# dbandstra/zang

Hardware: AMD Instinct MI355X
Metric: voice-samples/sec (higher is better)
Workload: dtype f32

## Files before the change

### zang_amd/csrc/common.hip.h

```cpp
#pragma once
#if defined(__HIPCC_RTC__)
#define ZH_DEVICE_ONLY 1
#endif
#include <hip/hip_runtime.h>
#if !defined(ZH_DEVICE_ONLY)
#include <stdint.h>
#include <stddef.h>
#include <new>
#endif
#include "rtc_types.hip.h"
#include "../../include/zang_hip.h"

#if !defined(ZH_DEVICE_ONLY)
#include <utility>
#include <vector>
#include <functional>
#include <memory>
#include <string>
struct zh_flipper {
    uint64_t id;
    zh_ctx *ctx;
    uint32_t n;
    uint32_t *cnt[2];
    int cur;
// ... 17 lines not shown
    std::function<void(hipStream_t, float *const *, uint32_t)> launch;
    const char *kernel = nullptr;
};
struct zh_direct_item {
    std::function<void(hipStream_t, float *const *, uint32_t)> launch;
    std::vector<float *> imgs;
    const char *kernel;
};

struct zh_ctx {
    int device;
    hipStream_t stream;
    bool own_stream;
    uint32_t capture_flags;
    bool epoch_open;
    zh_co_batch co;
    uint32_t co_paints, co_launches;
    std::string last_form;
    bool form_fresh;
    float *mix_partials;
    size_t mix_partials_floats;
    std::vector<float *> mix_retired;
    uint32_t graphs_live;
    std::vector<struct zh_graph *> graphs;
    bool capturing;
    uint32_t capture_serial;
    std::vector<zh_flip_use> capture_log;
    std::vector<std::pair<std::string, uint32_t>> capture_kernels;
    int deferred_error = 0;
    std::vector<zh_direct_item> co_plan;
    bool co_plan_ok = true;
    uint32_t capture_launches = 0, co_plan_launches = 0;
    void *noise_jump;
};

struct zh_graph {
    zh_ctx *ctx;
    hipGraph_t graph;
    hipGraphExec_t exec;
    std::vector<zh_flip_use> flips;
    uint32_t nodes = 0;
    uint32_t co_paints = 0, co_launches = 0;
    std::vector<std::pair<std::string, uint32_t>> kernels;
    std::vector<zh_direct_item> plan;
    std::vector<std::pair<std::string, uint32_t>> plan_kernels;
};

struct ZhDeviceGuard {
    int prev, want;
    explicit ZhDeviceGuard(int device) : prev(-1), want(device) {
        if (want < 0) return;
        if (hipGetDevice(&prev) != hipSuccess) { prev = -1; return; }
        if (prev != want) (void)hipSetDevice(want);
    }
    ~ZhDeviceGuard() { if (want >= 0 && prev >= 0 && prev != want) (void)hipSetDevice(prev); }
    ZhDeviceGuard(const ZhDeviceGuard &) = delete;
    ZhDeviceGuard &operator=(const ZhDeviceGuard &) = delete;
};
void zh_epoch_barrier(zh_ctx *ctx);
extern thread_local zh_ctx *zh_tls_ctx;
struct ZhFormScope {
    zh_ctx *prev;
    explicit ZhFormScope(const zh_ctx *c) : prev(zh_tls_ctx) {
        if (!prev) { zh_tls_ctx = const_cast<zh_ctx *>(c); if (zh_tls_ctx) zh_tls_ctx->form_fresh = true; }
    }
    ~ZhFormScope() { zh_tls_ctx = prev; }
};
#define ZH_GUARD_EPOCH(ctxptr) const zh_ctx *_zh_gctx = (ctxptr); ZhDeviceGuard _zh_guard(_zh_gctx ? _zh_gctx->device : -1); ZhFormScope _zh_fscope(_zh_gctx)
#define ZH_LAUNCH(kernel, ...) do { zh_note_launch(zh_tls_ctx, #kernel); hipLaunchKernelGGL(kernel, __VA_ARGS__); } while (0)
#define ZH_GUARD(ctxptr) ZH_GUARD_EPOCH(ctxptr); do { if (_zh_gctx && _zh_gctx->epoch_open) zh_epoch_barrier(const_cast<zh_ctx *>(_zh_gctx)); } while (0)
void zh_epoch_flush_batch(zh_ctx *ctx, bool last);

void zh_flipper_register(zh_flipper *f);
void zh_flipper_unregister(zh_flipper *f);
void zh_flipper_used(zh_flipper *f);
void zh_flipper_painted(zh_flipper *f);

enum { ZF_SINE_RANGES, ZF_NOISE_RANGES, ZF_ENVELOPE_RANGES, ZF_SAMPLER_RANGES, ZF_DECIMATOR_RANGES, ZF_CURVE_RANGES, ZF_CYCLE_RANGES,
       ZF_PORTAMENTO_RANGES, ZF_PULSE_CTRL_RANGES, ZF_PULSE_CTRL_SUMS, ZF_TRISAW_CTRL_RANGES, ZF_TRISAW_CTRL_QUOT, ZF_PMOSC_RANGES,
       ZF_SCRIPT_RANGES, ZF_SCRIPT_RANGES_MAXV, ZF_OSC_FC, ZF_NICE_PC_MAX, ZF_NICE_PC4_MAX, ZF_NICE_WAVE_MAX, ZF_PMOSC_WAVE_MAX,
       ZF_NICE_MIX_ROLL, ZF_NICE_MIX_WG_MIN, ZF_NF_PC_MAX, ZF_NF_RING_MAX, ZF_FILTER_PC_MAX, ZF_FILTER_PC16_MAX, ZF_FILTER_PC_CTL_MAX,
       ZF_PINK_PIPE_MAX, ZF_PINK_TAPS, ZF_ECHOES_PC_MAX, ZF_DELAY_FRAMES_MAX, ZF_FILTER_TP_MAX, ZF_NF_TP_MAX, ZF_NICE_TP_MAX,
       ZF_PINK_TP_MAX, ZF_ECHOES_TP_MAX, ZF_NICE_MIX_FMA, ZF_BASICS_ROWS_MIN, ZF_SCRIPT_PC, ZF_SCRIPT_PC_MAXV, ZF_NF_TP_PIPE_FRAMES, ZF_DISTORTION_ROWS_MIN, ZF_DISTORTION_RC, ZF_GRAPH_DIRECT,
       ZF_STEREO_ECHOES_PC_MAX, ZF_COUNT };
long zh_form(int id);
bool zh_form_is_set(int id);
uint32_t zh_range_frames(uint32_t V, uint32_t n, int form, uint32_t target_waves, uint32_t max_voices);
void zh_note_launch(zh_ctx *ctx, const char *kernel);
extern thread_local const char *zh_tls_launch_detail;

constexpr int kMixGroupFrames = 8;

struct zh_event {
    hipEvent_t ev;
};
#endif

#define ZH_INLINE_LAMBDA __attribute__((always_inline))

#if !defined(ZH_DEVICE_ONLY)
#define ZH_TRY(expr)                                   \
    do {                                               \
        hipError_t _e = (expr);                        \
        if (_e != hipSuccess) return (int)_e;          \
    } while (0)

static inline int zh_launch_status() {
    hipError_t e = hipGetLastError();
    return e == hipSuccess ? ZH_OK : (int)e;
}
#endif

struct Img {
    float *p;
    uint32_t stride;
    __device__ __forceinline__ float *at(uint32_t f, uint32_t v) const { return p + (size_t)f * stride + v; }
};
struct CImg {
    const float *p;
    uint32_t stride;
    __device__ __forceinline__ const float *at(uint32_t f, uint32_t v) const { return p + (size_t)f * stride + v; }
};
struct F32P {
    float value;
    const float *pv;
    __device__ __forceinline__ float get(uint32_t v) const { return pv ? pv[v] : value; }
};
struct BoolP {
    uint32_t value;
    const uint8_t *pv;
    __device__ __forceinline__ bool get(uint32_t v) const { return pv ? pv[v] != 0 : value != 0; }
};
struct CobP {
    uint32_t is_buffer;
    F32P c;
    CImg b;
};

#if !defined(ZH_DEVICE_ONLY)
static inline Img mk_img(const zh_buf &b) { return Img{b.ptr, b.stride}; }
static inline CImg mk_cimg(const zh_buf &b) { return CImg{b.ptr, b.stride}; }
static inline F32P mk_f32(const zh_f32 &f) { return F32P{f.value, f.per_voice}; }
static inline BoolP mk_bool(const zh_bool &b) { return BoolP{b.value, b.per_voice}; }
static inline CobP mk_cob(const zh_cob &c) {
    return CobP{c.tag == ZH_COB_BUFFER ? 1u : 0u, mk_f32(c.constant), mk_cimg(c.buffer)};
}

constexpr uint32_t kMaxRowStride = 1u << 26;
static inline bool buf_covers(const zh_buf &b, uint32_t n_voices, uint32_t span_end) {
    return b.ptr != nullptr && b.voices >= n_voices && b.frames >= span_end && b.stride >= n_voices && b.stride <= kMaxRowStride;
}
static inline bool bufs_alias(const zh_buf &a, const zh_buf &b) {
    if (!a.ptr || !b.ptr) return false;
    const float *ae = a.ptr + (size_t)a.frames * a.stride, *be = b.ptr + (size_t)b.frames * b.stride;
    return a.ptr < be && b.ptr < ae;
}
static inline bool cob_aliases(const zh_cob &c, const zh_buf &b) { return c.tag == ZH_COB_BUFFER && bufs_alias(c.buffer, b); }
static inline int zh_zero_first_aliased(zh_ctx *ctx, uint32_t start, uint32_t end, const zh_buf &out, uint32_t n_voices, bool aliased, uint32_t &flags) {
    if (!aliased || !(flags & ZH_PAINT_ZERO_FIRST)) return ZH_OK;
    flags &= ~(uint32_t)ZH_PAINT_ZERO_FIRST;
    zh_buf o = out;
    o.voices = n_voices;
    return end > start ? zh_zero(ctx, start, end, o) : ZH_OK;
}
static inline bool cob_ok(const zh_cob &c, uint32_t n_voices, uint32_t span_end) {
    if (c.tag == ZH_COB_CONSTANT) return true;
    if (c.tag == ZH_COB_BUFFER) return buf_covers(c.buffer, n_voices, span_end);
// ... 59 lines not shown
```

### zang_amd/csrc/composite.hip

```cpp
#include "common.hip.h"
#include <memory>
#include "ring.hip.h"
#include "zmath.hip.h"
#include "dsp.hip.h"
#include "seq.hip.h"
#include "envelope.hip.h"
#include "voices.hip.h"
#include "span_walk.hip.h"
#include "noise_jump.hip.h"
#define ZH_FILTER_TP_NOISE 1
#include "filter_tp.hip.h"
#include <vector>
#include <string.h>
#include <stdlib.h>

int zh_mix_reserve(zh_ctx *ctx, size_t floats);
void zh_mix_pass2_launch(zh_ctx *ctx, uint32_t tiles, uint32_t nframes, float *dst, int zero_first);
void zh_mix_pass2_launch_at(zh_ctx *ctx, const float *partials, uint32_t tiles, uint32_t nframes, float *dst, int zero_first);
void zh_mix_pass2_wide_launch(zh_ctx *ctx, const float *partials, size_t channel_stride, uint32_t rows, uint32_t nframes, float *dst0,
                              float *dst1, int channels, int zero_first);
void zh_mix_pass2_wide_batch_launch(zh_ctx *ctx, const float *partials, size_t channel_stride, uint32_t rows, uint32_t nframes,
                                    float *const *dst0, float *const *dst1, uint32_t n_buffers, int channels, int zero_first);

struct zh_nice {
// ... 1218 lines not shown
    if (!m || !outputs || !p || end < start || !buf_covers(outputs[0], m->n, end)) return ZH_ERR_INVALID;
    if (m->n == 0) return ZH_OK;
    hipStream_t st = m->ctx->stream;
    NiceArgs a = nice_args(m, p, note_id_changed);
    const Img out = mk_img(outputs[0]);
    const bool zf = (flags & ZH_PAINT_ZERO_FIRST) != 0;
    if ((flags & ZH_PAINT_TOLERANT) && end - start >= 128 && end - start <= kNiceTpMaxChunks * 128u) {
        const uint32_t C = zh_tp_chunks(m->n, ZF_NICE_TP_MAX, end - start);
        if (C >= 2 && !m->tp && !m->ctx->capturing && dev_alloc(&m->tp, (size_t)kNiceTpWords * m->n) != ZH_OK) { m->tp = nullptr; (void)hipGetLastError(); }
        if (C >= 2 && m->tp) {
            NiceTpArgs t;
            t.a = a; t.tp = m->tp; t.start = start; t.end = end; t.L = ((end - start + C - 1) / C + 7) / 8 * 8; t.out = out;
            const dim3 grid((m->n + 255) / 256, (end - start + t.L - 1) / t.L);
            ZH_LAUNCH(k_nice_tp_a, grid, dim3(256), 0, st, t);
            if (zf) ZH_LAUNCH(k_nice_tp_b<true>, grid, dim3(256), 0, st, t);
            else ZH_LAUNCH(k_nice_tp_b<false>, grid, dim3(256), 0, st, t);
            return zh_launch_status();
        }
    }
    if (m->n <= nice_pc_max() && end > start && outputs[0].stride <= (1u << 24)) {
        const long pc4_max = zh_form(ZF_NICE_PC4_MAX);
        if ((long)m->n <= pc4_max) {
            if (zf) ZH_LAUNCH(k_nice_pc4<true>, seq_grid(m->n), dim3(256), 0, st, a, out, start, end);
            else ZH_LAUNCH(k_nice_pc4<false>, seq_grid(m->n), dim3(256), 0, st, a, out, start, end);
        } else {
            if (zf) ZH_LAUNCH(k_nice_pc<true>, seq_grid(m->n), dim3(192), 0, st, a, out, start, end);
            else ZH_LAUNCH(k_nice_pc<false>, seq_grid(m->n), dim3(192), 0, st, a, out, start, end);
        }
    } else {
        if (zf) ZH_LAUNCH((k_nice<true, 1>), seq_grid(m->n), dim3(kSeqBlock), 0, st, a, out, start, end);
        else ZH_LAUNCH((k_nice<false, 1>), seq_grid(m->n), dim3(kSeqBlock), 0, st, a, out, start, end);
    }
    return zh_launch_status();
}
static bool nice_mix_roll() { return zh_form(ZF_NICE_MIX_ROLL) != 0; }
static int nice_mix_wg(uint32_t n_voices) { return (long)n_voices >= zh_form(ZF_NICE_MIX_WG_MIN) ? 4 : 0; }
constexpr uint32_t kNiceCoalesceReserve = 8;
static int nice_paint_mix_n(zh_nice *m, uint32_t start, uint32_t end, float *mix_l, float *mix_r, const zh_f32 *gain_l,
                            const zh_f32 *gain_r, zh_bool note_id_changed, const zh_nice_params *p, uint32_t flags) {
    const bool stereo = mix_r != nullptr;
    if (!m || !mix_l || !p || end < start) return ZH_ERR_INVALID;
    if (m->n == 0) return ZH_OK;
    const uint32_t nframes = end - start;
    const int wg = nice_mix_wg(m->n);
    const uint32_t bs = 256u;
    const uint32_t blocks = (m->n + bs - 1) / bs;
    const uint32_t rows = wg ? blocks : blocks * 4;
    const size_t per_channel = (size_t)rows * kMixGroupFrames * ((nframes + kMixGroupFrames - 1) / kMixGroupFrames ? (nframes + kMixGroupFrames - 1) / kMixGroupFrames : 1);
    int rc = zh_mix_reserve(m->ctx, per_channel * (stereo ? 2 : 1) * (stereo && !m->ctx->capturing ? kNiceCoalesceReserve : 1u));
    if (rc) return rc;
    hipStream_t st = m->ctx->stream;
    NiceArgs a = nice_args(m, p, note_id_changed);
    float *part = m->ctx->mix_partials;
    const int zf = (int)(flags & ZH_PAINT_ZERO_FIRST);
    if ((flags & ZH_PAINT_TOLERANT) && !wg && nframes >= 128 && nframes <= kNiceTpMaxChunks * 128u) {
        const uint32_t Cn = zh_tp_chunks(m->n, ZF_NICE_TP_MAX, nframes);
        if (Cn >= 2 && !m->tp && !m->ctx->capturing && dev_alloc(&m->tp, (size_t)kNiceTpWords * m->n) != ZH_OK) { m->tp = nullptr; (void)hipGetLastError(); }
        if (Cn >= 2 && m->tp) {
            NiceTpArgs t;
            t.a = a; t.tp = m->tp; t.start = start; t.end = end; t.L = ((nframes + Cn - 1) / Cn + MIXF - 1) / MIXF * MIXF; t.out = Img{nullptr, 0};
            const dim3 grid(blocks, (nframes + t.L - 1) / t.L);
            ZH_LAUNCH(k_nice_tp_a, grid, dim3(256), 0, st, t);
            const bool roll = nice_mix_roll();
            if (stereo) {
                const F32P gl = mk_f32(*gain_l), gr = mk_f32(*gain_r);
                if (roll) ZH_LAUNCH((k_nice_mix_tp_b<2, true>), grid, dim3(256), 0, st, t, part, gl, gr);
                else ZH_LAUNCH((k_nice_mix_tp_b<2, false>), grid, dim3(256), 0, st, t, part, gl, gr);
                zh_mix_pass2_wide_launch(m->ctx, part, per_channel, rows, nframes, mix_l + start, mix_r + start, 2, zf);
            } else {
                const F32P none = mk_f32(zh_f32{0.0f, 0, nullptr});
                if (roll) ZH_LAUNCH((k_nice_mix_tp_b<1, true>), grid, dim3(256), 0, st, t, part, none, none);
                else ZH_LAUNCH((k_nice_mix_tp_b<1, false>), grid, dim3(256), 0, st, t, part, none, none);
                zh_mix_pass2_wide_launch(m->ctx, part, per_channel, rows, nframes, mix_l + start, nullptr, 1, zf);
            }
            return zh_launch_status();
        }
    }
    if ((flags & ZH_PAINT_TOLERANT) && zh_form(ZF_NICE_MIX_FMA) != 0) {
        const F32P none = mk_f32(zh_f32{0.0f, 0, nullptr});
        zh_nice_mix_fma_launch(stereo ? 2 : 1, nice_mix_roll(), wg, blocks, st, a, start, end, part, stereo ? mk_f32(*gain_l) : none, stereo ? mk_f32(*gain_r) : none);
        if (nframes) zh_mix_pass2_wide_launch(m->ctx, part, per_channel, rows, nframes, mix_l + start, stereo ? mix_r + start : nullptr, stereo ? 2 : 1, zf);
        return zh_launch_status();
    }
#define ZH_NMIX(C_, ROLL_, NW_, GL_, GR_) ZH_LAUNCH((k_nice_mix<C_, ROLL_, NW_>), dim3(blocks), dim3(bs), 0, st, a, start, end, part, GL_, GR_)
#define ZH_NMIX_W(C_, ROLL_, GL_, GR_) do { if (wg) ZH_NMIX(C_, ROLL_, 4, GL_, GR_); else ZH_NMIX(C_, ROLL_, 0, GL_, GR_); } while (0)
    const bool roll = nice_mix_roll();
    if (stereo) {
        const F32P gl = mk_f32(*gain_l), gr = mk_f32(*gain_r);
        if (roll) ZH_NMIX_W(2, true, gl, gr); else ZH_NMIX_W(2, false, gl, gr);
        if (nframes) zh_mix_pass2_wide_launch(m->ctx, part, per_channel, rows, nframes, mix_l + start, mix_r + start, 2, zf);
    } else {
        const F32P none = mk_f32(zh_f32{0.0f, 0, nullptr});
        if (roll) ZH_NMIX_W(1, true, none, none); else ZH_NMIX_W(1, false, none, none);
        if (nframes) zh_mix_pass2_wide_launch(m->ctx, part, per_channel, rows, nframes, mix_l + start, nullptr, 1, zf);
    }
#undef ZH_NMIX_W
#undef ZH_NMIX
    return zh_launch_status();
}
int zh_nice_paint_mix(zh_nice *m, uint32_t start, uint32_t end, float *mix, zh_bool note_id_changed,
                      const zh_nice_params *p, uint32_t flags) { ZH_GUARD(m ? m->ctx : nullptr);
    return nice_paint_mix_n(m, start, end, mix, nullptr, nullptr, nullptr, note_id_changed, p, flags);
}
constexpr uint32_t kNiceCoalesceMax = 8;
static int nice_paint_mix_batch_impl(zh_nice *m, uint32_t start, uint32_t end, uint32_t n_buffers, float *const *mix_left,
                                     float *const *mix_right, zh_f32 gain_left, zh_f32 gain_right, const zh_bool *note_id_changed,
                                     const zh_nice_params *params, uint32_t flags);
struct NiceHeld { float *l, *r; zh_bool nic; zh_nice_params p; };
struct NiceHeldBatch { std::vector<NiceHeld> v; zh_f32 gl, gr; uint32_t flags, sample_rate_bits; };
static bool same_f32(const zh_f32 &a, const zh_f32 &b) {
    return a.per_voice == b.per_voice && (a.per_voice || __builtin_bit_cast(uint32_t, a.value) == __builtin_bit_cast(uint32_t, b.value));
}
int zh_nice_paint_mix_stereo(zh_nice *m, uint32_t start, uint32_t end, float *mix_left, float *mix_right, zh_f32 gain_left,
                             zh_f32 gain_right, zh_bool note_id_changed, const zh_nice_params *p, uint32_t flags) { ZH_GUARD_EPOCH(m ? m->ctx : nullptr);
    if (!mix_right) return ZH_ERR_INVALID;
    zh_ctx *ctx = m ? m->ctx : nullptr;
    const bool hold = ctx && ctx->capturing && (ctx->capture_flags & ZH_CAPTURE_COALESCE) && mix_left && p && end > start && m->n &&
                      (!(flags & ZH_PAINT_TOLERANT) || nice_mix_wg(m->n));
    bool fits = false;
    if (hold) {
        const uint32_t blocks = (m->n + 255u) / 256u, rows = nice_mix_wg(m->n) ? blocks : blocks * 4;
        const uint32_t groups = (end - start + kMixGroupFrames - 1) / kMixGroupFrames;
        fits = (size_t)rows * kMixGroupFrames * groups * 2 <= ctx->mix_partials_floats;
    }
    if (!hold || !fits) {
        if (ctx && ctx->epoch_open) zh_epoch_barrier(ctx);
        return nice_paint_mix_n(m, start, end, mix_left, mix_right, &gain_left, &gain_right, note_id_changed, p, flags);
    }
    zh_co_batch &cb = ctx->co;
    std::shared_ptr<NiceHeldBatch> held = cb.active && cb.owner == m ? std::static_pointer_cast<NiceHeldBatch>(cb.items) : nullptr;
    const uint32_t sr_bits = __builtin_bit_cast(uint32_t, p->sample_rate);
    bool join = held && cb.start == start && cb.end == end && held->flags == flags && held->sample_rate_bits == sr_bits && held->v.size() < kNiceCoalesceMax &&
                same_f32(held->gl, gain_left) && same_f32(held->gr, gain_right);
    for (size_t q = 0; join && q < held->v.size(); q++) {
        const float *rows[2] = {held->v[q].l, held->v[q].r};
        for (const float *x : rows)
            if ((mix_left < x + end && x < mix_left + end) || (mix_right < x + end && x < mix_right + end)) join = false;
    }
    if (!join) {
        zh_epoch_flush_batch(ctx, false);
        held = std::make_shared<NiceHeldBatch>();
        held->gl = gain_left; held->gr = gain_right; held->flags = flags; held->sample_rate_bits = sr_bits;
        cb.items = held;
        cb.active = true; cb.owner = m; cb.start = start; cb.end = end; cb.stride = 0; cb.key = 0; cb.flips = false;
        ctx->epoch_open = true;
        std::shared_ptr<NiceHeldBatch> items = held;
        cb.launch = [m, start, end, gain_left, gain_right, flags, items](hipStream_t, float *const *, uint32_t cnt) {
            const std::vector<NiceHeld> &v = items->v;
            float *l[kNiceCoalesceMax], *r[kNiceCoalesceMax];
            zh_bool nic[kNiceCoalesceMax];
            zh_nice_params ps[kNiceCoalesceMax];
            for (uint32_t i = 0; i < cnt; i++) { l[i] = v[i].l; r[i] = v[i].r; nic[i] = v[i].nic; ps[i] = v[i].p; }
            int rc = cnt > 1 ? nice_paint_mix_batch_impl(m, start, end, cnt, l, r, gain_left, gain_right, nic, ps, flags) : ZH_ERR_UNSUPPORTED;
            if (rc != ZH_OK) {
                for (uint32_t i = 0; i < cnt; i++) {
                    rc = nice_paint_mix_n(m, start, end, l[i], r[i], &gain_left, &gain_right, nic[i], &ps[i], flags);
                    if (rc != ZH_OK && !m->ctx->deferred_error) m->ctx->deferred_error = rc;
                }
            }
        };
    }
    held->v.push_back(NiceHeld{mix_left, mix_right, note_id_changed, *p});
    cb.imgs.push_back(mix_left);
    ctx->co_paints++;
    return ZH_OK;
}

static int nice_paint_mix_batch_impl(zh_nice *m, uint32_t start, uint32_t end, uint32_t n_buffers, float *const *mix_left,
                                     float *const *mix_right, zh_f32 gain_left, zh_f32 gain_right, const zh_bool *note_id_changed,
                                     const zh_nice_params *params, uint32_t flags) {
    if (!m || !mix_left || !mix_right || !note_id_changed || !params || end < start || n_buffers > (uint32_t)kNiceMixMaxBatch) return ZH_ERR_INVALID;
    for (uint32_t k = 0; k < n_buffers; k++) {
        if (!mix_left[k] || !mix_right[k]) return ZH_ERR_INVALID;
        if (__builtin_bit_cast(uint32_t, params[k].sample_rate) != __builtin_bit_cast(uint32_t, params[0].sample_rate)) return ZH_ERR_UNSUPPORTED;
    }
    if (m->n == 0 || n_buffers == 0) return ZH_OK;
    const uint32_t nframes = end - start;
    const int wg = nice_mix_wg(m->n);
    const uint32_t bs = 256u;
    const uint32_t blocks = (m->n + bs - 1) / bs, rows = wg ? blocks : blocks * 4;
    const size_t per_channel = (size_t)rows * kMixGroupFrames * ((nframes + kMixGroupFrames - 1) / kMixGroupFrames ? (nframes + kMixGroupFrames - 1) / kMixGroupFrames : 1);
    int rc = zh_mix_reserve(m->ctx, per_channel * 2 * n_buffers);
    if (rc) return rc;
    NiceBatchArgs b;
    b.a = nice_args(m, &params[0], note_id_changed[0]);
    b.nb = n_buffers;
    for (int k = 0; k < kNiceMixMaxBatch; k++) {
        const uint32_t j = (uint32_t)k < n_buffers ? (uint32_t)k : 0u;
        b.freq[k] = mk_f32(params[j].freq); b.note_on[k] = mk_bool(params[j].note_on); b.nic[k] = mk_bool(note_id_changed[j]);
    }
    float *part = m->ctx->mix_partials;
    hipStream_t st = m->ctx->stream;
#define ZH_NMIXB(ROLL_, NW_) ZH_LAUNCH((k_nice_mix_batch<2, ROLL_, NW_>), dim3(blocks), dim3(bs), 0, st, b, start, end, part, mk_f32(gain_left), mk_f32(gain_right))
    if ((flags & ZH_PAINT_TOLERANT) && zh_form(ZF_NICE_MIX_FMA) != 0)
        zh_nice_mix_batch_fma_launch(nice_mix_roll(), wg, blocks, st, b, start, end, part, mk_f32(gain_left), mk_f32(gain_right));
    else if (wg) { if (nice_mix_roll()) ZH_NMIXB(true, 4); else ZH_NMIXB(false, 4); }
    else { if (nice_mix_roll()) ZH_NMIXB(true, 0); else ZH_NMIXB(false, 0); }
#undef ZH_NMIXB
    if (nframes) {
        float *l[kNiceMixMaxBatch], *r[kNiceMixMaxBatch];
        for (uint32_t k = 0; k < n_buffers; k++) { l[k] = mix_left[k] + start; r[k] = mix_right[k] + start; }
        zh_mix_pass2_wide_batch_launch(m->ctx, part, per_channel, rows, nframes, l, r, n_buffers, 2, (int)(flags & ZH_PAINT_ZERO_FIRST));
    }
    return zh_launch_status();
}

int zh_nice_paint_mix_stereo_batch(zh_nice *m, uint32_t start, uint32_t end, uint32_t n_buffers, float *const *mix_left,
                                   float *const *mix_right, zh_f32 gain_left, zh_f32 gain_right, const zh_bool *note_id_changed,
                                   const zh_nice_params *params, uint32_t flags) { ZH_GUARD(m ? m->ctx : nullptr);
    return nice_paint_mix_batch_impl(m, start, end, n_buffers, mix_left, mix_right, gain_left, gain_right, note_id_changed, params, flags);
}

static bool span_table_ok(const zh_span_table *t) {
    return t && t->max_spans > 0 && t->count && t->start && t->end && t->freq && t->note_on && t->note_id_changed;
}
static SpanTableP mk_span_table(const zh_span_table *t) {
    return SpanTableP{t->max_spans, t->count, t->start, t->end, t->freq, t->note_on, t->note_id_changed};
}

int zh_nice_paint_spans(zh_nice *m, uint32_t start, uint32_t end, const zh_buf *outputs, const zh_buf *temps,
                        float sample_rate, const zh_span_table *table, uint32_t flags) { ZH_GUARD(m ? m->ctx : nullptr);
    (void)temps;
    if (!m || !outputs || end < start || !buf_covers(outputs[0], m->n, end) || !span_table_ok(table)) return ZH_ERR_INVALID;
    if (m->n == 0) return ZH_OK;
    hipStream_t st = m->ctx->stream;
    zh_nice_params p;
    memset(&p, 0, sizeof p);
    p.sample_rate = sample_rate;
    zh_bool no = {0, 0, nullptr};
    NiceArgs a = nice_args(m, &p, no);
    const bool zf = (flags & ZH_PAINT_ZERO_FIRST) != 0;
    const long wave_max = zh_form(ZF_NICE_WAVE_MAX);
    if ((long)m->n <= wave_max) {
        if (zf) ZH_LAUNCH(k_nice_spans_wave<true>, dim3(m->n), dim3(64), 0, st, a, mk_span_table(table), mk_img(outputs[0]), start, end);
        else ZH_LAUNCH(k_nice_spans_wave<false>, dim3(m->n), dim3(64), 0, st, a, mk_span_table(table), mk_img(outputs[0]), start, end);
    } else if (zf) ZH_LAUNCH(k_nice_spans<true>, seq_grid(m->n), dim3(kSeqBlock), 0, st, a, mk_span_table(table), mk_img(outputs[0]), start, end);
    else ZH_LAUNCH(k_nice_spans<false>, seq_grid(m->n), dim3(kSeqBlock), 0, st, a, mk_span_table(table), mk_img(outputs[0]), start, end);
    return zh_launch_status();
}

int zh_noise_filter_create(zh_ctx *ctx, uint32_t n, uint64_t first_seed, zh_noise_filter **out) { ZH_GUARD(ctx);
    if (!ctx || !out) return ZH_ERR_INVALID;
    zh_noise_filter *m = new (std::nothrow) zh_noise_filter();
    if (!m) return ZH_ERR_INVALID;
    memset(m, 0, sizeof *m);
    m->ctx = ctx; m->n = n;
    int rc = 0;
    for (int i = 0; i < 4 && !rc; i++) rc = dev_alloc(&m->s[i], n);
    if (!rc) rc = dev_alloc(&m->nb, (size_t)7 * n);
    if (!rc) rc = dev_alloc(&m->l, n);
    if (!rc) rc = dev_alloc(&m->b, n);
    if (!rc) rc = dev_alloc(&m->err, 1);
    if (!rc) rc = (int)hipMemsetAsync(m->err, 0, 4, ctx->stream);
    if (!rc && n) {
        rc = (int)hipMemsetAsync(m->nb, 0, (size_t)7 * n * 4, ctx->stream);
        if (!rc) rc = (int)hipMemsetAsync(m->l, 0, (size_t)n * 4, ctx->stream);
        if (!rc) rc = (int)hipMemsetAsync(m->b, 0, (size_t)n * 4, ctx->stream);
    }
    if (rc) { nf_free(m); delete m; return rc; }
    if (n) ZH_LAUNCH(k_nf_seed, dim3((n + 255) / 256), dim3(256), 0, ctx->stream, m->s[0], m->s[1], m->s[2], m->s[3], n, first_seed);
    if (n) (void)zh_noise_jump_tables(ctx);
    *out = m;
    return zh_launch_status();
}
int zh_noise_filter_destroy(zh_noise_filter *m) { ZH_GUARD(m ? m->ctx : nullptr);
    if (!m) return ZH_ERR_INVALID;
    (void)hipStreamSynchronize(m->ctx->stream);
    nf_free(m);
    delete m;
// ... 309 lines not shown
```

### zang_amd/csrc/dispatch.hip

```cpp
#include "common.hip.h"
#include <mutex>
#include <stdlib.h>
#include <string.h>
#include <string>

namespace {
struct FormRow { const char *name; long def; const char *doc; };
const FormRow kForms[ZF_COUNT] = {
     {"sine_ranges", -1, "SineOsc: frame ranges of the span at once, each replaying the phase walk before it (k_sineosc_ranges); auto: ~4,096 waves up to 1 Mi voices, ~2,048 up to 65,536 with a control image"},
     {"noise_ranges", -1, "Noise: frame ranges from jumped generator states (noise_jump.hip); auto: by voice count up to 65,536"},
     {"envelope_ranges", -1, "Envelope: frame ranges, each replaying the clock (k_envelope_ranges); auto: ~2,048 waves up to 40,960 voices"},
     {"sampler_ranges", -1, "Sampler: frame ranges (positions are a product, no replay); auto: ~16,384 waves up to 1 Mi voices"},
     {"decimator_ranges", -1, "Decimator: frame ranges replaying the hold counter; auto: ~1,024-2,048 waves up to 65,536 voices"},
     {"curve_ranges", -1, "Curve: frame ranges; auto: ~2,048 waves up to 40,960 voices"},
     {"cycle_ranges", -1, "Cycle: frame ranges (constant speed); auto: ~1,024 waves up to 16,384 voices"},
     {"portamento_ranges", -1, "Portamento: frame ranges; auto: ~2,048 waves up to 32,768 voices"},
     {"pulse_ctrl_ranges", -1, "PulseOsc with a frequency image: frame ranges over the summed phase advances; auto: ~2,048 waves up to 40,960 voices"},
     {"pulse_ctrl_sums", 1, "... 1: a first kernel sums each range's own advances (k_pulseosc_ctrl_sums), 0: every range replays the frames before it"},
     {"trisaw_ctrl_ranges", -1, "TriSawOsc with a frequency image: frame ranges; auto: ~1,024 waves up to 16,384 voices"},
     {"trisaw_ctrl_quot", 1, "... 1: freq / sample_rate painted once into a module-owned image first (k_div_image), 0: divided in every replay"},
     {"pmosc_ranges", -1, "PMOscInstrument: frame ranges (k_pmosc_ranges); auto: ~2,048-4,096 waves up to 131,072 voices"},
     {"script_ranges", -1, "generated script kernels: frame ranges for modules without a delay ring; auto: by voice count"},
     {"script_ranges_maxv", 131072, "... the largest voice count that takes them"},
     {"osc_fc", 0, "constant-frequency PulseOsc / TriSawOsc: frames per lane of the chunked kernel; 0 = PulseOsc 4, from 16,384 voices 3 with non-temporal stores (profiles/r05/osc_large_voice_counts.txt); TriSawOsc 8-64 by voice count (tools/sweep_osc_fc.sh), PulseOsc's when the paint is a sawtooth for every voice (one color <= 0)"},
     {"nice_pc_max", 65536, "NiceInstrument: up to here the oscillator, envelope and filter chains run in three waves side by side (k_nice_pc: 72 vs 146 us at 4,096 voices, 107 vs 168 at 65,536; slower at 131,072)"},
     {"nice_pc4_max", 32768, "... and up to here in four (k_nice_pc4: 44 / 47 / 53.5 us at 4,096 / 16,384 / 32,768 voices against 60.5 / 62.5 / 63)"},
     {"nice_wave_max", 64, "zh_nice_paint_spans: up to here one WAVE per voice, lanes = frames (k_nice_spans_wave)"},
     {"pmosc_wave_max", 64, "zh_pmosc_paint_spans: the same (k_pmosc_spans_wave)"},
     {"nice_mix_roll", 1, "fused mixdown: the oscillator's half-period bit carried as a lane mask (1) or recomputed (0): 148.2 vs 149.6 us at 131,072 voices"},
     {"nice_mix_wg_min", 65536, "fused mixdown: from here one partial row per 256-voice workgroup instead of per wave (a quarter of the partial traffic; 4,096 voices: 99 -> 105 us with it, 131,072: level)"},
     {"nf_pc_max", 65536, "Noise -> Filter voice: up to here noise and filter in two waves side by side (k_noise_filter_pc: 75 vs 110 us at 4,096 voices, 111 vs 133 at 65,536)"},
     {"nf_ring_max", 16384, "... white noise: up to here three producer waves, a filter wave and a writer wave per 64 voices (k_noise_filter_ring)"},
     {"filter_pc_max", 32768, "Filter, constant cutoff / resonance: up to here the three-wave pipeline over 32-frame tiles (k_filter_pc: 41-51 us against 54-76 in one wave); 0 = never (the 16-frame form too unless filter_pc16_max is given), 1 = the 16-frame form only"},
     {"filter_pc16_max", 65536, "... 16-frame tiles above filter_pc_max up to here (36,864 / 65,536 voices: 72 / 104 us against 97 / 116)"},
     {"filter_pc_ctl_max", 32768, "... with control images (k_filter_pc_ctl: 47-98 us against 96-140 up to 32,768 voices)"},
     {"pink_pipe_max", 32768, "pink Noise: up to here white frame ranges + the taps as a second kernel (k_pink_taps / k_pink_pipe) instead of one loop"},
     {"pink_taps", 1, "... 1: four-wave tap kernel (32-frame tiles up to 16,384 voices, 16 above), 16: the 16-frame tiles always, 0: the seven-stage chain k_pink_pipe"},
     {"echoes_pc_max", 65536, "FilteredEchoes: up to here ring reader / filter / writer as waves side by side (k_filtered_echoes_pc)"},
     {"delay_frames_max", 4294967295, "Delay: up to here the frames of a delay length at once instead of the walk (57 -> 13 us at 4,096 voices, 423 -> 271 at 131,072: every voice count)"},
     {"filter_tp_max", 16384, "ZH_PAINT_TOLERANT Filter: the largest voice count painted as chunks at once (filter_tp.hip.h)"},
     {"nf_tp_max", 16384, "... Noise -> Filter voice"},
     {"nice_tp_max", 16384, "... NiceInstrument and its fused mixdown"},
     {"pink_tp_max", 16384, "... pink Noise"},
     {"echoes_tp_max", 6144, "... FilteredEchoes (six image streams: level with the exact form at 8,192 voices)"},
     {"nice_mix_fma", 1, "ZH_PAINT_TOLERANT fused mixdown above nice_tp_max voices: 1 = the kernel compiled with multiply-adds fused (nice_mix_fma.hip), 0 = the exact kernel"},
     {"basics_rows_min", 32768, "basics.zig operations (zero, set, copy, add ..., multiply ...): from here three consecutive rows of a 256-voice column per wave (k_elementwise_chunks) instead of the row-striding loop: 131,072 voices 12-23 % faster"},
     {"script_pc", -1, "generated script kernels: the role-wave form (zs_paint_pc_<name>: the body's builtin calls as producer / recurrence / writer waves over LDS tiles); auto: where the emitter found the lane form unable to take frame ranges and the longest role well below the whole body; 0 = never, 1 = every module that has the form"},
     {"script_pc_maxv", 65536, "... the largest voice count that takes it -- half of it for a module whose role form does more than 1.25 x the body's work or needs more than 9 waves (FilteredSawtooth: 53 / 57 / 66 / 110 us at 4,096 / 16,384 / 32,768 / 65,536 voices against 172-181 in one wave per 64 voices; slower at 131,072)"},
     {"nf_tp_pipe_frames", 0, "ZH_PAINT_TOLERANT Noise -> Filter voice recorded pipelined (ZH_CAPTURE_COALESCE, k_nf_tp_ba): frames per chunk, a multiple of 32; 0 = as outside a pipeline (32 at 4,096 voices)"},
     {"distortion_rows_min", 32768, "Distortion clip: from here four voices per lane, three consecutive rows of a 256-voice column per wave, the per-voice constants once per workgroup through LDS (k_distortion_chunks: 224 -> 178 us at 131,072 voices); the overdrive too when this row is set by hand (no faster: 239 against 244-250 us)"},
     {"distortion_rc", 0, "... rows per wave of that form: 3 (0), 6 or 8"},
     {"graph_direct", 1, "zh_graph_launch of a ZH_CAPTURE_COALESCE capture that recorded nothing but held-back oscillator batches: 1 = their launches enqueued directly, one per batch of up to 32 buffers (20 paints: one launch of 20), 0 = the recorded hipGraph (20 paints: two launches of 10)"},
     {"stereo_echoes_pc_max", 32768, "StereoEchoes: up to here loader / filter / writer waves (k_stereo_echoes_pc); StereoEchoes(15000), 1,024 frames, role waves against the walk: 253 / 318 us at 32,768 voices, 518 / 454 at 65,536 (profiles/r10)"},
};

struct Overrides { bool set[ZF_COUNT]; long val[ZF_COUNT]; };
Overrides parse_forms() {
    Overrides o;
    memset(&o, 0, sizeof o);
    const char *e = getenv("ZH_FORMS");
    if (!e) return o;
    std::string s(e);
    size_t i = 0;
    while (i < s.size()) {
        size_t j = s.find(',', i);
        if (j == std::string::npos) j = s.size();
        const std::string item = s.substr(i, j - i);
        const size_t eq = item.find('=');
        if (eq != std::string::npos) {
            const std::string name = item.substr(0, eq);
            for (int k = 0; k < ZF_COUNT; k++)
                if (name == kForms[k].name) { o.set[k] = true; o.val[k] = strtol(item.c_str() + eq + 1, nullptr, 10); }
        }
        i = j + 1;
    }
    return o;
}
}

bool zh_form_is_set(int id) {
    if (id < 0 || id >= ZF_COUNT) return false;
    return parse_forms().set[id];
}

long zh_form(int id) {
    if (id < 0 || id >= ZF_COUNT) return 0;
    static const bool live = [] { const char *e = getenv("ZH_ENV_LIVE"); return e && e[0] == '1'; }();
    if (live) {
        const Overrides o = parse_forms();
        return o.set[id] ? o.val[id] : kForms[id].def;
    }
    static const Overrides once = parse_forms();
    return once.set[id] ? once.val[id] : kForms[id].def;
}

uint32_t zh_range_frames(uint32_t V, uint32_t n, int form, uint32_t target_waves, uint32_t max_voices) {
    const long forced = zh_form(form);
    if (forced == 0 || V == 0 || n < 128 || V > max_voices) return 0;
    const uint32_t waves = (V + 63) / 64;
    uint32_t want = forced > 0 ? (uint32_t)forced : target_waves / waves;
    if (want < 2) return 0;
    if (want > 64) want = 64;
    const uint32_t ch = ((n + want - 1) / want + 7) / 8 * 8;
    return (n + ch - 1) / ch >= 2 ? ch : 0;
}

thread_local const char *zh_tls_launch_detail = nullptr;

void zh_note_launch(zh_ctx *ctx, const char *kernel) {
    const char *detail = zh_tls_launch_detail;
    zh_tls_launch_detail = nullptr;
    if (!ctx) return;
    if (ctx->capturing) {
        ctx->capture_launches++;
        const char *b0 = kernel;
        while (*b0 == '(' || *b0 == ' ') b0++;
        size_t n0 = 0;
        while (b0[n0] && b0[n0] != '<' && b0[n0] != ')' && b0[n0] != ' ') n0++;
        std::string key(b0, n0);
        if (detail) { key += '['; key += detail; key += ']'; }
        bool found = false;
        for (auto &kv : ctx->capture_kernels) if (kv.first == key) { kv.second++; found = true; break; }
        if (!found && ctx->capture_kernels.size() < 64) ctx->capture_kernels.emplace_back(key, 1u);
    }
    std::string &f = ctx->last_form;
    if (ctx->form_fresh) { f.clear(); ctx->form_fresh = false; }
    if (f.size() > 480) return;
    const char *b = kernel;
    while (*b == '(' || *b == ' ') b++;
    size_t n = 0;
    while (b[n] && b[n] != '<' && b[n] != ')' && b[n] != ' ') n++;
    if (!f.empty()) {
        const size_t last = f.rfind(',');
        const std::string prev = last == std::string::npos ? f : f.substr(last + 1);
        if (prev.compare(0, std::string::npos, b, n) == 0) return;
        f += ',';
// ... 28 lines not shown
```

### zang_amd/csrc/nice_mix.hip.h

```cpp
#pragma once
#include "nice.hip.h"
#ifndef ZH_K
#define ZH_K(name) name
#endif
constexpr int MIXF = 32;
constexpr int MIXS = 68;

template <int C, class G2>
__device__ __forceinline__ void nice_mix_gains(G2 &g2, const F32P &gain_l, const F32P &gain_r, bool live, uint32_t v, uint32_t wave, uint32_t rh) {
    typedef float f2 __attribute__((ext_vector_type(2)));
    if constexpr (C == 2) {
        __shared__ f2 gains[512];
        gains[threadIdx.x] = live ? f2{gain_l.get(v), gain_r.get(v)} : f2{0.0f, 0.0f};
        __syncthreads();
        const f2 *mine = &gains[wave * 64 + rh * 32];
#pragma unroll
        for (int j = 0; j < 32; j++) g2[j] = mine[j];
    }
}

template <int C, bool ROLL, int NW, class G2>
__device__ __forceinline__ void nice_mix_frames(NiceLane &n, PulseRoll &roll, const G2 &g2, float (*tile)[MIXS], float *__restrict__ pw_paint,
                                                size_t channel_stride, uint32_t rows, uint32_t wrow, uint32_t start, uint32_t end, uint32_t lane,
                                                uint32_t rf, uint32_t rh, float (*wsum)[NW ? NW : 4][C][MIXF] = nullptr, uint32_t wave = 0, uint32_t first = 0xFFFFFFFFu) {
    constexpr bool WG = NW != 0;
    uint32_t parity = 0;
    for (uint32_t f0 = first == 0xFFFFFFFFu ? start : first; f0 < end; f0 += MIXF) {
        const bool whole = f0 + MIXF <= end;
        if (!__any(n.env.mode == ENV_MODE_TOWARD)) {
            const float e0 = n.env_quiet();
            if (whole) {
#pragma unroll 4
                for (int k = 0; k < MIXF; k++) {
                    const float x = 0.0f + (ROLL ? n.template frame_quiet_roll<true>(e0, roll) : n.template frame_quiet<true>(e0));
                    tile[k][lane] = x;
                }
            } else {
                for (int k = 0; k < MIXF; k++) {
                    float x = 0.0f;
                    if (__builtin_amdgcn_readfirstlane((int)(f0 + k < end))) x = 0.0f + (ROLL ? n.template frame_quiet_roll<true>(e0, roll) : n.template frame_quiet<true>(e0));
                    tile[k][lane] = x;
                }
            }
        } else if (whole && n.env.quiet(MIXF)) {
            if (__all(n.env.mode == ENV_MODE_TOWARD)) {
#pragma unroll 4
                for (int k = 0; k < MIXF; k++) {
                    const float e0 = n.env.frame_masked_all_toward_quiet();
                    const float x = 0.0f + (ROLL ? n.template frame_quiet_roll<true>(e0, roll) : n.template frame_quiet<true>(e0));
                    tile[k][lane] = x;
                }
            } else {
#pragma unroll 4
                for (int k = 0; k < MIXF; k++) {
                    const float e0 = n.env.frame_masked_quiet();
                    const float x = 0.0f + (ROLL ? n.template frame_quiet_roll<true>(e0, roll) : n.template frame_quiet<true>(e0));
                    tile[k][lane] = x;
                }
            }
        } else if (whole) {
#pragma unroll 4
            for (int k = 0; k < MIXF; k++) {
                const float x = 0.0f + (ROLL ? n.template frame_roll<true>(roll) : n.template frame<true>());
                tile[k][lane] = x;
            }
        } else {
            for (int k = 0; k < MIXF; k++) {
                float x = 0.0f;
                if (__builtin_amdgcn_readfirstlane((int)(f0 + k < end))) x = 0.0f + (ROLL ? n.template frame_roll<true>(roll) : n.template frame<true>());
                tile[k][lane] = x;
            }
        }
        __builtin_amdgcn_fence(__ATOMIC_RELEASE, "wavefront");
        __builtin_amdgcn_wave_barrier();
        __builtin_amdgcn_fence(__ATOMIC_ACQUIRE, "wavefront");
        {
            const float4 *row4 = reinterpret_cast<const float4 *>(&tile[rf][rh * 32]);
            float row[32];
#pragma unroll
            for (int q = 0; q < 8; q++) { const float4 x = row4[q]; row[4 * q] = x.x; row[4 * q + 1] = x.y; row[4 * q + 2] = x.z; row[4 * q + 3] = x.w; }
            float sl, sr = 0.0f;
            if constexpr (C == 1) {
                sl = row[0];
#pragma unroll
                for (int j = 1; j < 32; j++) sl += row[j];
            } else {
                sl = row[0] * g2[0].x; sr = row[0] * g2[0].y;
#pragma unroll
                for (int j = 1; j < 32; j++) { sl += row[j] * g2[j].x; sr += row[j] * g2[j].y; }
            }
            const float hl = __shfl_down(sl, 32);
            const float hr = C == 2 ? __shfl_down(sr, 32) : 0.0f;
            if constexpr (!WG) {
                if (rh == 0 && f0 + rf < end) {
                    const uint32_t fr = (f0 - start) + rf;
                    float *pw = pw_paint + ((size_t)(fr / kMixGroupFrames) * rows + wrow) * kMixGroupFrames + (fr % kMixGroupFrames);
                    pw[0] = sl + hl;
                    if constexpr (C == 2) pw[channel_stride] = sr + hr;
                }
            } else {
                if (rh == 0) {
                    wsum[parity][wave][0][rf] = sl + hl;
                    if constexpr (C == 2) wsum[parity][wave][1][rf] = sr + hr;
                }
                __syncthreads();
                constexpr uint32_t FW = MIXF / (NW ? NW : 4);
                static_assert(kMixGroupFrames % FW == 0, "a wave's frames stay inside one frame group");
                const uint32_t q = lane % FW, c = lane / FW, fw = wave * FW + q;
                if (c < (uint32_t)C && f0 + fw < end) {
                    float t = wsum[parity][0][c][fw] + wsum[parity][1][c][fw];
#pragma unroll
                    for (int w = 2; w < (NW ? NW : 4); w++) t += wsum[parity][w][c][fw];
                    const uint32_t fr = (f0 - start) + fw;
                    pw_paint[c * channel_stride + ((size_t)(fr / kMixGroupFrames) * rows + wrow) * kMixGroupFrames + (fr % kMixGroupFrames)] = t;
                }
                parity ^= 1u;
            }
        }
        __builtin_amdgcn_fence(__ATOMIC_RELEASE, "wavefront");
        __builtin_amdgcn_wave_barrier();
    }
}

__device__ __forceinline__ void nice_silence(NiceLane &n) {
    n.k.ifreq = 0u; n.k.brpt = 0u; n.k.gdf2 = 0.0f; n.k.cc121 = 0.0f; n.k.cc212 = 0.0f; n.g = n.ng = 0.0f;
    n.l = n.b = 0.0f;
    n.env.mode = ENV_MODE_NONE; n.env.m_painted = 0u;
}

template <int C, bool ROLL, int NW = 0>
__global__ void __launch_bounds__(NW == 8 ? 512 : 256) ZH_K(k_nice_mix)(NiceArgs a, uint32_t start, uint32_t end, float *__restrict__ partials,
                                                                  F32P gain_l, F32P gain_r) {
    constexpr bool WG = NW != 0;
    constexpr int NWV = NW ? NW : 4;
    __shared__ float tile_all[NWV][MIXF][MIXS];
    __shared__ float wsum[WG ? 2 : 1][NWV][C][MIXF];
    const uint32_t v = blockIdx.x * (NWV * 64) + threadIdx.x;
    const uint32_t lane = threadIdx.x & 63, wave = threadIdx.x >> 6;
    float (*tile)[MIXS] = tile_all[wave];
    const uint32_t nframes = end - start;
    const uint32_t wave_global = WG ? blockIdx.x : blockIdx.x * NWV + wave;
    const uint32_t rows = WG ? gridDim.x : gridDim.x * NWV;
    const size_t channel_stride = (size_t)((nframes + kMixGroupFrames - 1) / kMixGroupFrames) * rows * kMixGroupFrames;
    const bool live = v < a.V;
    NiceLane n;
    nice_load(n, a, live ? v : a.V - 1);
    if (!live) nice_silence(n);
    const uint32_t rf = lane & (MIXF - 1), rh = lane >> 5;
    PulseRoll roll;
    n.roll_begin(roll);
    typedef float f2 __attribute__((ext_vector_type(2)));
    f2 g2[C == 2 ? 32 : 1];
    nice_mix_gains<C>(g2, gain_l, gain_r, live, v, wave, rh);
    nice_mix_frames<C, ROLL, NW>(n, roll, g2, tile, partials, channel_stride, rows, wave_global, start, end, lane, rf, rh, wsum, wave);
    if (live) nice_store(n, a, v);
}

constexpr int kNiceMixMaxBatch = 16;
struct NiceBatchArgs {
    NiceArgs a;
    F32P freq[kNiceMixMaxBatch];
    BoolP note_on[kNiceMixMaxBatch], nic[kNiceMixMaxBatch];
    uint32_t nb;
};
template <int C, bool ROLL, int NW = 0>
__global__ void __launch_bounds__(NW == 8 ? 512 : 256) ZH_K(k_nice_mix_batch)(const NiceBatchArgs b, uint32_t start, uint32_t end, float *__restrict__ partials,
                                                                        F32P gain_l, F32P gain_r) {
    constexpr bool WG = NW != 0;
    constexpr int NWV = NW ? NW : 4;
    __shared__ float tile_all[NWV][MIXF][MIXS];
    __shared__ float wsum[WG ? 2 : 1][NWV][C][MIXF];
    const NiceArgs &a = b.a;
    const uint32_t v = blockIdx.x * (NWV * 64) + threadIdx.x;
    const uint32_t lane = threadIdx.x & 63, wave = threadIdx.x >> 6;
    float (*tile)[MIXS] = tile_all[wave];
    const uint32_t nframes = end - start;
    const uint32_t wave_global = WG ? blockIdx.x : blockIdx.x * NWV + wave;
    const uint32_t rows = WG ? gridDim.x : gridDim.x * NWV;
    const size_t channel_stride = (size_t)((nframes + kMixGroupFrames - 1) / kMixGroupFrames) * rows * kMixGroupFrames;
    const bool live = v < a.V;
    const uint32_t vc = live ? v : a.V - 1;
    NiceLane n;
    nice_load_state(n, a, vc);
    const float color = a.color[vc];
    const uint32_t rf = lane & (MIXF - 1), rh = lane >> 5;
    typedef float f2 __attribute__((ext_vector_type(2)));
    f2 g2[C == 2 ? 32 : 1];
    nice_mix_gains<C>(g2, gain_l, gain_r, live, v, wave, rh);
    for (uint32_t k = 0; k < b.nb; k++) {
        n.begin(a.sample_rate, a.srf, a.sr8, b.freq[k].get(vc), color, b.note_on[k].get(vc), b.nic[k].get(vc));
        if (!live) nice_silence(n);
        PulseRoll roll;
        n.roll_begin(roll);
        nice_mix_frames<C, ROLL, NW>(n, roll, g2, tile, partials + (size_t)k * C * channel_stride, channel_stride, rows, wave_global, start, end, lane, rf, rh, wsum, wave);
    }
    if (live) nice_store(n, a, v);
}

void zh_nice_mix_fma_launch(int channels, bool roll, int nw, uint32_t blocks, hipStream_t st, const NiceArgs &a, uint32_t start, uint32_t end,
                            float *part, F32P gl, F32P gr);
void zh_nice_mix_batch_fma_launch(bool roll, int nw, uint32_t blocks, hipStream_t st, const NiceBatchArgs &bt, uint32_t start, uint32_t end,
                                  float *part, F32P gl, F32P gr);
```

### zang_amd/csrc/nice_mix_fma.hip

```cpp
#define ZH_K(name) name##_fma
#include "nice_mix.hip.h"

void zh_nice_mix_fma_launch(int channels, bool roll, int nw, uint32_t blocks, hipStream_t st, const NiceArgs &a, uint32_t start, uint32_t end,
                            float *part, F32P gl, F32P gr) {
    const dim3 g(blocks), b(256);
#define ZH_ONE(C_, ROLL_, NW_) ZH_LAUNCH((k_nice_mix_fma<C_, ROLL_, NW_>), g, b, 0, st, a, start, end, part, gl, gr)
#define ZH_ROLL(C_, NW_) do { if (roll) ZH_ONE(C_, true, NW_); else ZH_ONE(C_, false, NW_); } while (0)
    if (channels == 2) { if (nw) ZH_ROLL(2, 4); else ZH_ROLL(2, 0); }
    else { if (nw) ZH_ROLL(1, 4); else ZH_ROLL(1, 0); }
#undef ZH_ROLL
#undef ZH_ONE
}

void zh_nice_mix_batch_fma_launch(bool roll, int nw, uint32_t blocks, hipStream_t st, const NiceBatchArgs &bt, uint32_t start, uint32_t end,
                                  float *part, F32P gl, F32P gr) {
    const dim3 g(blocks), b(256);
#define ZH_ONE(ROLL_, NW_) ZH_LAUNCH((k_nice_mix_batch_fma<2, ROLL_, NW_>), g, b, 0, st, bt, start, end, part, gl, gr)
    if (nw) { if (roll) ZH_ONE(true, 4); else ZH_ONE(false, 4); }
    else { if (roll) ZH_ONE(true, 0); else ZH_ONE(false, 0); }
#undef ZH_ONE
}
```

Measured before the change: 1702 billion.

## Compute wave-uniform envelope once per chunk across lanes in nice mix

Adds a path to the fused nice mixdown kernels that checks, with a ballot, whether all 64 voices in a wave carry identical envelope state. If they do, the envelope values for a 32-frame chunk are computed once, spread across lanes, written to a per-wave shared row and read back as float4. Otherwise every lane keeps computing its own envelope. The aim is to remove redundant per-lane envelope arithmetic for chords that share one note_on, at the cost of a uniformity check, extra LDS and wave barriers.

```diff
diff --git a/zang_amd/csrc/common.hip.h b/zang_amd/csrc/common.hip.h
--- a/zang_amd/csrc/common.hip.h
+++ b/zang_amd/csrc/common.hip.h
@@ -123,7 +123,7 @@
        ZF_NICE_MIX_ROLL, ZF_NICE_MIX_WG_MIN, ZF_NF_PC_MAX, ZF_NF_RING_MAX, ZF_FILTER_PC_MAX, ZF_FILTER_PC16_MAX, ZF_FILTER_PC_CTL_MAX,
        ZF_PINK_PIPE_MAX, ZF_PINK_TAPS, ZF_ECHOES_PC_MAX, ZF_DELAY_FRAMES_MAX, ZF_FILTER_TP_MAX, ZF_NF_TP_MAX, ZF_NICE_TP_MAX,
        ZF_PINK_TP_MAX, ZF_ECHOES_TP_MAX, ZF_NICE_MIX_FMA, ZF_BASICS_ROWS_MIN, ZF_SCRIPT_PC, ZF_SCRIPT_PC_MAXV, ZF_NF_TP_PIPE_FRAMES, ZF_DISTORTION_ROWS_MIN, ZF_DISTORTION_RC, ZF_GRAPH_DIRECT,
-       ZF_STEREO_ECHOES_PC_MAX, ZF_COUNT };
+       ZF_STEREO_ECHOES_PC_MAX, ZF_NICE_ENV_SHARED, ZF_COUNT };
 long zh_form(int id);
 bool zh_form_is_set(int id);
 uint32_t zh_range_frames(uint32_t V, uint32_t n, int form, uint32_t target_waves, uint32_t max_voices);
diff --git a/zang_amd/csrc/composite.hip b/zang_amd/csrc/composite.hip
--- a/zang_amd/csrc/composite.hip
+++ b/zang_amd/csrc/composite.hip
@@ -1324,9 +1324,10 @@
         if (nframes) zh_mix_pass2_wide_launch(m->ctx, part, per_channel, rows, nframes, mix_l + start, stereo ? mix_r + start : nullptr, stereo ? 2 : 1, zf);
         return zh_launch_status();
     }
-#define ZH_NMIX(C_, ROLL_, NW_, GL_, GR_) ZH_LAUNCH((k_nice_mix<C_, ROLL_, NW_>), dim3(blocks), dim3(bs), 0, st, a, start, end, part, GL_, GR_)
+#define ZH_NMIX(C_, ROLL_, NW_, GL_, GR_) ZH_LAUNCH((k_nice_mix<C_, ROLL_, NW_>), dim3(blocks), dim3(bs), 0, st, a, start, end, part, GL_, GR_, env_shared)
 #define ZH_NMIX_W(C_, ROLL_, GL_, GR_) do { if (wg) ZH_NMIX(C_, ROLL_, 4, GL_, GR_); else ZH_NMIX(C_, ROLL_, 0, GL_, GR_); } while (0)
     const bool roll = nice_mix_roll();
+    const uint32_t env_shared = zh_form(ZF_NICE_ENV_SHARED) != 0 ? 1u : 0u;
     if (stereo) {
         const F32P gl = mk_f32(*gain_l), gr = mk_f32(*gain_r);
         if (roll) ZH_NMIX_W(2, true, gl, gr); else ZH_NMIX_W(2, false, gl, gr);
@@ -1427,6 +1428,7 @@
     NiceBatchArgs b;
     b.a = nice_args(m, &params[0], note_id_changed[0]);
     b.nb = n_buffers;
+    b.env_shared = zh_form(ZF_NICE_ENV_SHARED) != 0 ? 1u : 0u;
     for (int k = 0; k < kNiceMixMaxBatch; k++) {
         const uint32_t j = (uint32_t)k < n_buffers ? (uint32_t)k : 0u;
         b.freq[k] = mk_f32(params[j].freq); b.note_on[k] = mk_bool(params[j].note_on); b.nic[k] = mk_bool(note_id_changed[j]);
diff --git a/zang_amd/csrc/dispatch.hip b/zang_amd/csrc/dispatch.hip
--- a/zang_amd/csrc/dispatch.hip
+++ b/zang_amd/csrc/dispatch.hip
@@ -52,6 +52,7 @@
      {"distortion_rc", 0, "... rows per wave of that form: 3 (0), 6 or 8"},
      {"graph_direct", 1, "zh_graph_launch of a ZH_CAPTURE_COALESCE capture that recorded nothing but held-back oscillator batches: 1 = their launches enqueued directly, one per batch of up to 32 buffers (20 paints: one launch of 20), 0 = the recorded hipGraph (20 paints: two launches of 10)"},
      {"stereo_echoes_pc_max", 32768, "StereoEchoes: up to here loader / filter / writer waves (k_stereo_echoes_pc); StereoEchoes(15000), 1,024 frames, role waves against the walk: 253 / 318 us at 32,768 voices, 518 / 454 at 65,536 (profiles/r10)"},
+     {"nice_env_shared", 1, "fused mixdown (exact kernels): a wave whose 64 voices hold one envelope -- a chord that got one note_on -- computes a chunk's envelope values once, frames across lanes (EnvLane::block64), instead of in every lane; same bits; 0 = never"},
 };
 
 struct Overrides { bool set[ZF_COUNT]; long val[ZF_COUNT]; };
diff --git a/zang_amd/csrc/nice_mix.hip.h b/zang_amd/csrc/nice_mix.hip.h
--- a/zang_amd/csrc/nice_mix.hip.h
+++ b/zang_amd/csrc/nice_mix.hip.h
@@ -5,6 +5,20 @@
 #endif
 constexpr int MIXF = 32;
 constexpr int MIXS = 68;
+#ifndef ZH_NICE_ENV_SHARED
+#define ZH_NICE_ENV_SHARED 1
+#endif
+constexpr bool kNiceEnvShared = ZH_NICE_ENV_SHARED != 0;
+constexpr int MIXE = 64;
+
+__device__ __forceinline__ bool nice_env_uniform(const NiceLane &n, bool live) {
+    const auto dif_u = [](uint32_t x) { return x ^ (uint32_t)__builtin_amdgcn_readfirstlane((int)x); };
+    const auto dif_f = [&](float x) { return dif_u(__builtin_bit_cast(uint32_t, x)); };
+    const auto &e = n.env;
+    const uint32_t dif = dif_u(e.state) | dif_f(e.t) | dif_f(e.last_value) | dif_f(e.start) | dif_u(e.mode) | dif_f(e.cur_step) | dif_f(e.cur_goal) |
+                         dif_f(e.cur_delta) | dif_u(e.m_painted) | dif_u(e.note_on ? 1u : 0u);
+    return __builtin_amdgcn_ballot_w64(live && dif == 0u) == ~0ull;
+}
 
 template <int C, class G2>
 __device__ __forceinline__ void nice_mix_gains(G2 &g2, const F32P &gain_l, const F32P &gain_r, bool live, uint32_t v, uint32_t wave, uint32_t rh) {
@@ -22,7 +36,8 @@
 template <int C, bool ROLL, int NW, class G2>
 __device__ __forceinline__ void nice_mix_frames(NiceLane &n, PulseRoll &roll, const G2 &g2, float (*tile)[MIXS], float *__restrict__ pw_paint,
                                                 size_t channel_stride, uint32_t rows, uint32_t wrow, uint32_t start, uint32_t end, uint32_t lane,
-                                                uint32_t rf, uint32_t rh, float (*wsum)[NW ? NW : 4][C][MIXF] = nullptr, uint32_t wave = 0, uint32_t first = 0xFFFFFFFFu) {
+                                                uint32_t rf, uint32_t rh, float (*wsum)[NW ? NW : 4][C][MIXF] = nullptr, uint32_t wave = 0, uint32_t first = 0xFFFFFFFFu,
+                                                bool shared = false, float *erow = nullptr) {
     constexpr bool WG = NW != 0;
     uint32_t parity = 0;
     for (uint32_t f0 = first == 0xFFFFFFFFu ? start : first; f0 < end; f0 += MIXF) {
@@ -39,6 +54,35 @@
                 for (int k = 0; k < MIXF; k++) {
                     float x = 0.0f;
                     if (__builtin_amdgcn_readfirstlane((int)(f0 + k < end))) x = 0.0f + (ROLL ? n.template frame_quiet_roll<true>(e0, roll) : n.template frame_quiet<true>(e0));
+                    tile[k][lane] = x;
+                }
+            }
+        } else if (kNiceEnvShared && shared) {
+            const float e = n.env.block64(whole ? (uint32_t)MIXF : end - f0, lane, erow);
+            __builtin_amdgcn_fence(__ATOMIC_RELEASE, "wavefront");
+            __builtin_amdgcn_wave_barrier();
+            if (lane < (uint32_t)MIXF) erow[lane] = e;
+            __builtin_amdgcn_fence(__ATOMIC_RELEASE, "wavefront");
+            __builtin_amdgcn_wave_barrier();
+            __builtin_amdgcn_fence(__ATOMIC_ACQUIRE, "wavefront");
+            const float4 *e4 = reinterpret_cast<const float4 *>(erow);
+            if (whole) {
+                for (int q = 0; q < MIXF / 4; q++) {
+                    const float4 ev = e4[q];
+                    const float e0[4] = {ev.x, ev.y, ev.z, ev.w};
+#pragma unroll
+                    for (int j = 0; j < 4; j++) {
+                        const float x = 0.0f + (ROLL ? n.template frame_quiet_roll<true>(e0[j], roll) : n.template frame_quiet<true>(e0[j]));
+                        tile[4 * q + j][lane] = x;
+                    }
+                }
+            } else {
+                for (int k = 0; k < MIXF; k++) {
+                    float x = 0.0f;
+                    if (__builtin_amdgcn_readfirstlane((int)(f0 + k < end))) {
+                        const float e0 = erow[k];
+                        x = 0.0f + (ROLL ? n.template frame_quiet_roll<true>(e0, roll) : n.template frame_quiet<true>(e0));
+                    }
                     tile[k][lane] = x;
                 }
             }
@@ -130,10 +174,11 @@
 
 template <int C, bool ROLL, int NW = 0>
 __global__ void __launch_bounds__(NW == 8 ? 512 : 256) ZH_K(k_nice_mix)(NiceArgs a, uint32_t start, uint32_t end, float *__restrict__ partials,
-                                                                  F32P gain_l, F32P gain_r) {
+                                                                  F32P gain_l, F32P gain_r, uint32_t env_shared) {
     constexpr bool WG = NW != 0;
     constexpr int NWV = NW ? NW : 4;
     __shared__ float tile_all[NWV][MIXF][MIXS];
+    __shared__ float erow_all[kNiceEnvShared ? NWV : 1][MIXE];
     __shared__ float wsum[WG ? 2 : 1][NWV][C][MIXF];
     const uint32_t v = blockIdx.x * (NWV * 64) + threadIdx.x;
     const uint32_t lane = threadIdx.x & 63, wave = threadIdx.x >> 6;
@@ -152,7 +197,9 @@
     typedef float f2 __attribute__((ext_vector_type(2)));
     f2 g2[C == 2 ? 32 : 1];
     nice_mix_gains<C>(g2, gain_l, gain_r, live, v, wave, rh);
-    nice_mix_frames<C, ROLL, NW>(n, roll, g2, tile, partials, channel_stride, rows, wave_global, start, end, lane, rf, rh, wsum, wave);
+    const bool shared = kNiceEnvShared && env_shared != 0u && nice_env_uniform(n, live);
+    nice_mix_frames<C, ROLL, NW>(n, roll, g2, tile, partials, channel_stride, rows, wave_global, start, end, lane, rf, rh, wsum, wave, 0xFFFFFFFFu,
+                                 shared, erow_all[kNiceEnvShared ? wave : 0]);
     if (live) nice_store(n, a, v);
 }
 
@@ -162,6 +209,7 @@
     F32P freq[kNiceMixMaxBatch];
     BoolP note_on[kNiceMixMaxBatch], nic[kNiceMixMaxBatch];
     uint32_t nb;
+    uint32_t env_shared;
 };
 template <int C, bool ROLL, int NW = 0>
 __global__ void __launch_bounds__(NW == 8 ? 512 : 256) ZH_K(k_nice_mix_batch)(const NiceBatchArgs b, uint32_t start, uint32_t end, float *__restrict__ partials,
@@ -169,6 +217,7 @@
     constexpr bool WG = NW != 0;
     constexpr int NWV = NW ? NW : 4;
     __shared__ float tile_all[NWV][MIXF][MIXS];
+    __shared__ float erow_all[kNiceEnvShared ? NWV : 1][MIXE];
     __shared__ float wsum[WG ? 2 : 1][NWV][C][MIXF];
     const NiceArgs &a = b.a;
     const uint32_t v = blockIdx.x * (NWV * 64) + threadIdx.x;
@@ -192,7 +241,9 @@
         if (!live) nice_silence(n);
         PulseRoll roll;
         n.roll_begin(roll);
-        nice_mix_frames<C, ROLL, NW>(n, roll, g2, tile, partials + (size_t)k * C * channel_stride, channel_stride, rows, wave_global, start, end, lane, rf, rh, wsum, wave);
+        const bool shared = kNiceEnvShared && b.env_shared != 0u && nice_env_uniform(n, live);
+        nice_mix_frames<C, ROLL, NW>(n, roll, g2, tile, partials + (size_t)k * C * channel_stride, channel_stride, rows, wave_global, start, end, lane, rf, rh, wsum, wave,
+                                     0xFFFFFFFFu, shared, erow_all[kNiceEnvShared ? wave : 0]);
     }
     if (live) nice_store(n, a, v);
 }
diff --git a/zang_amd/csrc/nice_mix_fma.hip b/zang_amd/csrc/nice_mix_fma.hip
--- a/zang_amd/csrc/nice_mix_fma.hip
+++ b/zang_amd/csrc/nice_mix_fma.hip
@@ -1,10 +1,11 @@
 #define ZH_K(name) name##_fma
+#define ZH_NICE_ENV_SHARED 0
 #include "nice_mix.hip.h"
 
 void zh_nice_mix_fma_launch(int channels, bool roll, int nw, uint32_t blocks, hipStream_t st, const NiceArgs &a, uint32_t start, uint32_t end,
                             float *part, F32P gl, F32P gr) {
     const dim3 g(blocks), b(256);
-#define ZH_ONE(C_, ROLL_, NW_) ZH_LAUNCH((k_nice_mix_fma<C_, ROLL_, NW_>), g, b, 0, st, a, start, end, part, gl, gr)
+#define ZH_ONE(C_, ROLL_, NW_) ZH_LAUNCH((k_nice_mix_fma<C_, ROLL_, NW_>), g, b, 0, st, a, start, end, part, gl, gr, 0u)
 #define ZH_ROLL(C_, NW_) do { if (roll) ZH_ONE(C_, true, NW_); else ZH_ONE(C_, false, NW_); } while (0)
     if (channels == 2) { if (nw) ZH_ROLL(2, 4); else ZH_ROLL(2, 0); }
     else { if (nw) ZH_ROLL(1, 4); else ZH_ROLL(1, 0); }
```

Measured after the change: 1661 billion. 0.976x the previous value.
